# derinworks/penr-oz-neural-network-torch

Hardware: AMD Instinct MI355X
Metric: training samples/sec (whole node), 4x8192 MLP bf16 at 1/2/4/8 MI355X (higher is better)
Workload: dtype bf16; 1 GPU; model=mlp[1024,4096,4096,1024] relu,relu,softmax (25.2M params), global_batch=8192, per_gpu_batch=8192, parallelism=dp1, optimizer=adam, dist_backend=none, dist_world_size=1, launcher=none, config_key=mlp4, engine=fused, grad_dtype=bf16

## Files before the change

penr_oz_neural_network_torch_amd/csrc/bindings.cpp:

```cpp
#include <fcntl.h>
#include <sys/mman.h>
#include <sys/stat.h>
#include <unistd.h>
#include <ATen/ATen.h>
#include <c10/hip/HIPStream.h>
#include <algorithm>
#include <map>
#include <mutex>

#include <torch/library.h>

#include <cstdint>
#include <cstdio>
#include <cstring>
#include <limits>
#include <tuple>
#include <vector>

#include "gemm_dispatch.h"
#include "gemm_sk_plan.h"
#include "json_format.h"
#include "pz_kernels.h"

namespace {
// ... 552 lines not shown
}

void stage_fwd_op(const Tensor& x, const Tensor& y, at::IntArrayRef ei, at::ArrayRef<double> ef) {
  check_dev(x, "x");
  TORCH_CHECK(x.is_contiguous() && y.is_contiguous() && x.numel() == y.numel(), "pz::stage_fwd: contiguous x/y");
  PZ_HIP_CHECK(pz::stage_fwd(x.data_ptr(), dt_of(x), y.data_ptr(), dt_of(y), x.numel(), make_epi(ei, ef), cur_stream(x)));
}

void stage_bwd_op(const Tensor& g, const Tensor& y, const Tensor& dx, at::IntArrayRef ei, at::ArrayRef<double> ef) {
  check_dev(g, "g");
  TORCH_CHECK(g.is_contiguous() && y.is_contiguous() && dx.is_contiguous(), "pz::stage_bwd: contiguous tensors");
  TORCH_CHECK(g.scalar_type() == y.scalar_type() && g.scalar_type() == dx.scalar_type(), "pz::stage_bwd: dtypes");
  TORCH_CHECK(y.is_cuda() && dx.is_cuda() && y.numel() == g.numel() && dx.numel() == g.numel(),
              "pz::stage_bwd: g, y and dx must be GPU tensors of one size");
  PZ_HIP_CHECK(pz::stage_bwd(g.data_ptr(), y.data_ptr(), dx.data_ptr(), dt_of(g), g.numel(), make_epi(ei, ef),
                             cur_stream(g)));
}

void xent_head_op(const Tensor& logits, const Tensor& labels, int64_t rows_valid, const optional<Tensor>& loss,
                  double loss_scale, const optional<Tensor>& dh, double grad_scale, const optional<Tensor>& colsum,
                  const optional<Tensor>& probs, at::IntArrayRef ei, at::ArrayRef<double> ef, int64_t idx_ld,
                  const optional<Tensor>& out8, const optional<Tensor>& out8_qscale, const optional<Tensor>& amax,
                  bool store_dh, const optional<Tensor>& su_amax, const optional<Tensor>& su_qs, double su_headroom,
                  double su_maxval, const optional<Tensor>& su_qs_prev) {
  check_dev(logits, "logits");
  TORCH_CHECK(logits.dim() == 2 && logits.stride(1) == 1, "pz::xent_head: 2-D logits");
  TORCH_CHECK(labels.scalar_type() == at::kLong && labels.is_contiguous(), "pz::xent_head: int64 labels");
  pz::XentArgs a{};
  a.logits = logits.data_ptr();
  a.ld = logits.stride(0);
  a.labels = labels.data_ptr<int64_t>();
  a.rows = static_cast<int>(logits.size(0));
  TORCH_CHECK(rows_valid >= 0 && rows_valid <= logits.size(0), "pz::xent_head: rows_valid ", rows_valid,
              " is outside [0, ", logits.size(0), "]");
  TORCH_CHECK(labels.is_cuda() && labels.numel() >= rows_valid, "pz::xent_head: labels must hold rows_valid entries");
  a.rows_valid = static_cast<int>(rows_valid);
  a.cols = static_cast<int>(logits.size(1));
  a.dtype = dt_of(logits);
  head_accumulators(a, loss, colsum, a.dtype == pz::DT_F64, "pz::xent_head");
  at::Tensor cs_ws;
  if (a.colsum != nullptr && a.dtype == pz::DT_BF16 && pz::deterministic()) {
    const int blocks = (a.rows + 31) / 32, groups = (blocks + 15) / 16;
    cs_ws = at::empty({static_cast<int64_t>(blocks + groups) * a.cols}, logits.options().dtype(at::kFloat));
    a.cs_ws = cs_ws.data_ptr<float>();
    a.cs_tickets = split_counters(groups + 1, logits.device());
  }
  a.loss_scale = loss_scale;
  if (dh.has_value() && dh->defined()) {
    a.dh = opt_mat(dh, logits, a.rows, a.cols, "pz::xent_head", "dh");
// ... 6 lines not shown
  }
  a.epi = make_epi(ei, ef);
  a.idx_ld = idx_ld > 0 ? idx_ld : a.cols;
  if (out8.has_value() && out8->defined()) {
    TORCH_CHECK(out8->scalar_type() == at::kFloat8_e5m2 && out8->dim() == 2 && out8->stride(1) == 1 &&
                    out8->size(0) >= a.rows && out8->size(1) >= a.cols,
                "pz::xent_head: out8 must be float8_e5m2 [rows, cols]");
    a.out8 = static_cast<uint8_t*>(out8->data_ptr());
    a.ld_out8 = out8->stride(0);
    a.out8_qscale = f32_scalar_ptr(out8_qscale, "out8_qscale");
    TORCH_CHECK(a.out8_qscale != nullptr, "pz::xent_head: out8 needs out8_qscale");
    a.amax = opt_vec<float>(amax, at::kFloat, 1, "pz::xent_head", "amax");
  }
  a.skip_dh = store_dh ? 0 : 1;
  a.su = scale_upd(su_amax, su_qs, su_headroom, su_maxval);
  if (su_qs_prev.has_value() && su_qs_prev->defined()) {
    TORCH_CHECK(a.su.n > 0 && su_qs_prev->scalar_type() == at::kFloat && su_qs_prev->is_contiguous() &&
                    su_qs_prev->numel() >= 2 * a.su.n && su_qs_prev->data_ptr<float>() != a.su.qs,
                "pz::xent_head: su_qs_prev: fp32 qs[2n] of the current step, not su_qs itself");
    a.su.qs_prev = su_qs_prev->data_ptr<float>();
  }
  TORCH_CHECK((a.out8 == nullptr && !a.skip_dh) || pz::xent_head_out8_ok(a),
              "pz::xent_head: out8 / store_dh=False need the bf16 fast path (bf16, cols % 8 == 0, <= 2048, aligned)");
  PZ_HIP_CHECK(pz::xent_head(a, cur_stream(logits)));
}

void mse_head_op(const Tensor& y, const Tensor& target, int64_t rows_valid, const optional<Tensor>& loss,
                 double loss_scale, const optional<Tensor>& dh, double grad_scale, const optional<Tensor>& colsum,
                 at::IntArrayRef ei, at::ArrayRef<double> ef, int64_t idx_ld) {
  check_dev(y, "y");
  TORCH_CHECK(y.dim() == 2 && target.dim() == 2 && y.stride(1) == 1 && target.stride(1) == 1, "pz::mse_head: 2-D");
  TORCH_CHECK(y.scalar_type() == target.scalar_type(), "pz::mse_head: dtype mismatch");
  TORCH_CHECK(rows_valid >= 0 && rows_valid <= y.size(0), "pz::mse_head: rows_valid ", rows_valid, " is outside [0, ",
              y.size(0), "]");
  TORCH_CHECK(target.is_cuda() && target.size(0) >= rows_valid && target.size(1) >= y.size(1),
              "pz::mse_head: target must hold [rows_valid, cols]");
  pz::MseArgs a{};
  a.y = y.data_ptr();
  a.ld_y = y.stride(0);
  a.target = target.data_ptr();
  a.ld_t = target.stride(0);
  a.rows = static_cast<int>(y.size(0));
  a.rows_valid = static_cast<int>(rows_valid);
  a.cols = static_cast<int>(y.size(1));
  a.dtype = dt_of(y);
  head_accumulators(a, loss, colsum, a.dtype == pz::DT_F64, "pz::mse_head");
  a.loss_scale = loss_scale;
// ... 762 lines not shown
        "Tensor(a!) params, Tensor(b!)? exp_avg, Tensor(c!)? exp_avg_sq, Tensor(d!)? shadow, Tensor(e!)? stats, "
        "Tensor(f!)? amax, bool adam, float lr, float beta1, float beta2, float eps, float bias_c1, "
        "float bias_c2_sqrt, float grad_scale, float l2, Tensor? hp=None, Tensor? epoch=None, int stats_every=1) -> ()");
  m.def("gemm_path(Tensor A, bool a_kc, Tensor B, bool b_kc, Tensor C, int M, int N, int K, "
        "bool force_generic=False) -> int");
  m.def("gemm_skinny(Tensor x, Tensor w, Tensor(a!) out, Tensor? bias, int act) -> ()");
  m.def("gemm_skinny_eligible(Tensor x, Tensor w, Tensor out) -> bool");
  m.def("gemm_skinny_w8(Tensor x, Tensor w8, Tensor scale, Tensor(a!) out, Tensor? bias, int act) -> ()");
  m.def("gemm_skinny_w8_eligible(Tensor x, Tensor w8, Tensor scale, Tensor out) -> bool");
  m.def("gemm_skinny_plan(int K, int N, int dtype) -> int[]");
  m.def("gemm_skinny_w8_plan(int K, int N) -> int[]");
  m.def("gemm_sk_plan(int M, int N, int K, int cus, int M1=0, int N1=0) -> int[]");
  m.def("gemm_pair_split(Tensor A0, Tensor B0, Tensor C0, Tensor A1, Tensor B1, Tensor C1, int M0, int N0, int M1, "
        "int N1, int K, int engine=0) -> int");
  m.def("gemm_pair(Tensor A0, Tensor B0, Tensor(a!) C0, Tensor A1, Tensor B1, Tensor(b!) C1, int M0, int N0, int M1, "
        "int N1, int K, Tensor? scale_a0=None, Tensor? scale_b0=None, Tensor? scale_a1=None, "
        "Tensor? scale_b1=None, int flags=0) -> ()");
  m.def("stage_fwd(Tensor x, Tensor(a!) y, int[] epi_i, float[] epi_f) -> ()");
  m.def("stage_bwd(Tensor g, Tensor y, Tensor(a!) dx, int[] epi_i, float[] epi_f) -> ()");
  m.def("xent_head(Tensor logits, Tensor labels, int rows_valid, Tensor(a!)? loss, float loss_scale, Tensor(b!)? dh, "
        "float grad_scale, Tensor(c!)? colsum, Tensor(d!)? probs, int[] epi_i, float[] epi_f, int idx_ld, "
        "Tensor(e!)? out8=None, Tensor? out8_qscale=None, Tensor(f!)? amax=None, bool store_dh=True, "
        "Tensor(s!)? su_amax=None, Tensor(t!)? su_qs=None, float su_headroom=1.0, float su_maxval=448.0, "
        "Tensor? su_qs_prev=None) -> ()");
  m.def("mse_head(Tensor y, Tensor target, int rows_valid, Tensor(a!)? loss, float loss_scale, Tensor(b!)? dh, "
        "float grad_scale, Tensor(c!)? colsum, int[] epi_i, float[] epi_f, int idx_ld) -> ()");
  m.def("softmax_rows(Tensor x, Tensor(a!) y) -> ()");
  m.def("sample_rows(Tensor logits, Tensor(a!) seq, Tensor(b!) done, int pos, float temperature, int top_k, int key, "
        "int stop_token=-1, int row0=0, float top_p=1.0, float min_p=0.0) -> ()");
  m.def("generate_resident(Tensor(a!) seq, Tensor(b!) done, Tensor[] params, int[] plan, int steps, float temperature, "
        "int top_k, int seed_lo, int seed_hi, int stop_token=-1, int row0=0, Tensor(c!)? logits_out=None, float top_p=1.0, "
        "float min_p=0.0) -> ()");
  m.def("token_logprob(Tensor logits, Tensor targets, Tensor(a!) logprob, Tensor(b!)? rank) -> ()");
  m.def("topk_rows(Tensor logits, int k, Tensor(a!) idx, Tensor(b!) logprob) -> ()");
  m.def("softmax_bwd(Tensor g, Tensor y, Tensor(a!) dx) -> ()");
  m.def("colsum(Tensor x, Tensor(a!) out) -> ()");
  m.def("gather_rows(Tensor data, Tensor? indices, int seed_lo, int seed_hi, Tensor(a!) out, int rows_valid, "
        "Tensor? labels_in, Tensor(b!)? labels_out, Tensor(c!)? picked, Tensor? epoch=None, Tensor? data8=None, "
        "Tensor(d!)? out8=None, Tensor(s!)? su_amax=None, Tensor(t!)? su_qs=None, float su_headroom=1.0, "
        "float su_maxval=448.0) -> ()");
  m.def("pack_segments(int[] offsets, int[] numels, int[] is_weight, int[] stat_slot, Tensor?[] shadows, "
        "Tensor?[] grads16, int[] zero_grad, Tensor?[] amax, Tensor?[] w8, Tensor?[] w8_amax_prev, "
        "Tensor?[] w8_qs) -> Tensor");
  m.def("optimizer_step(Tensor(a!) params, Tensor(e!) grads, Tensor(b!)? exp_avg, Tensor(c!)? exp_avg_sq, Tensor segments, "
        "Tensor block_seg, int num_segments, int total_blocks, bool adam, float lr, float beta1, float beta2, float eps, "
        "float bias_c1, float bias_c2_sqrt, float grad_scale, float l2, Tensor(d!)? stats, Tensor? hp=None, "
        "Tensor? epoch=None, int stats_every=1, int max_grid=0) -> ()");
// ... 82 lines not shown
```

penr_oz_neural_network_torch_amd/csrc/elementwise.hip:

```cpp
#include "pz_common.h"
#include "pz_launch.h"
#include "pz_kernels.h"

namespace pz {
namespace {

template <typename T> PZ_DEV double ldd(const T* p, int64_t i) { return static_cast<double>(p[i]); }
template <> PZ_DEV double ldd<uint16_t>(const uint16_t* p, int64_t i) { return bf2f(p[i]); }
template <typename T> PZ_DEV void std_(T* p, int64_t i, double v) { p[i] = static_cast<T>(v); }
template <> PZ_DEV void std_<uint16_t>(uint16_t* p, int64_t i, double v) { p[i] = f2bf(static_cast<float>(v)); }

template <typename Tin, typename Tout, typename F>
__global__ void __launch_bounds__(256) stage_fwd_kernel(const Tin* __restrict__ x, Tout* __restrict__ y,
                                                        int64_t n, EpiSpec e) {
  e = epi_resolve(e);
  for (int64_t i = blockIdx.x * int64_t(256) + threadIdx.x; i < n; i += int64_t(gridDim.x) * 256) {
    const F v = static_cast<F>(ldd<Tin>(x, i));
    std_<Tout>(y, i, static_cast<double>(epi_fwd<F>(v, static_cast<uint64_t>(i), e)));
  }
}

template <typename T, typename F>
__global__ void __launch_bounds__(256) stage_bwd_kernel(const T* __restrict__ g, const T* __restrict__ y,
                                                        T* __restrict__ dx, int64_t n, EpiSpec e) {
// ... 26 lines not shown
  if (threadIdx.x == 0) atomicAdd(loss + (slots > 1 ? blockIdx.x % slots : 0), red[0] + red[1] + red[2] + red[3]);
}

template <typename A>
PZ_DEV void block_colsum_flush(A* colsum, const A* cs, int cols) {
  __syncthreads();
  for (int c = threadIdx.x; c < cols; c += 256)
    if (cs[c] != A(0)) atomicAdd(colsum + c, cs[c]);
}

template <int WAVES>
PZ_DEV void head_colsum_flush(const XentArgs& a, const float* cs_lds) {
  __shared__ int det_flag;
  for (int c = threadIdx.x; c < a.cols; c += WAVES * 64) {
    float t = 0.f;
#pragma unroll
    for (int w = 0; w < WAVES; ++w) t += cs_lds[w * a.cols + c];
    if (a.cs_ws != nullptr) st_wt(a.cs_ws + static_cast<int64_t>(blockIdx.x) * a.cols + c, t);
    else if (t != 0.f) atomicAdd(a.colsum + c, t);
  }
  if (a.cs_ws != nullptr)
    det_colsum<WAVES * 64>(a.cs_ws, a.cs_tickets, gridDim.x, 16, blockIdx.x, a.cols, a.cols, a.colsum,
                           (PZ_LDS int*)(&det_flag));
}

template <typename F> PZ_DEV F* head_loss(void* f32, void* f64);
template <> PZ_DEV float* head_loss<float>(void* f32, void*) { return static_cast<float*>(f32); }
template <> PZ_DEV double* head_loss<double>(void*, void* f64) { return static_cast<double*>(f64); }

template <typename T, typename F>
__global__ void __launch_bounds__(256) xent_head_kernel(XentArgs a) {
  apply_scale_update(a.su);
  a.epi = epi_resolve(a.epi);
  extern __shared__ __attribute__((aligned(16))) char cs_raw[];
  F* cs_lds = reinterpret_cast<F*>(cs_raw);
  __shared__ F red[4];
  F* const loss = head_loss<F>(a.loss, a.loss64);
  F* const colsum = head_loss<F>(a.colsum, a.colsum64);
  const T* __restrict__ logits = static_cast<const T*>(a.logits);
  T* __restrict__ dh = static_cast<T*>(a.dh);
  T* __restrict__ probs = static_cast<T*>(a.probs);
  const int lane = threadIdx.x & 63;
  const int wave = threadIdx.x >> 6;
  const bool cs_on = colsum != nullptr && dh != nullptr;
  if (cs_on) {
    for (int c = threadIdx.x; c < a.cols; c += 256) cs_lds[c] = F(0);
// ... 279 lines not shown
  A s = A(0);
  if (c < cols)
    for (int r = r0 + (threadIdx.x >> 6); r < r1; r += 4) s += static_cast<A>(ldd<T>(x, static_cast<int64_t>(r) * ld + c));
  __shared__ A part[4][64];
  part[threadIdx.x >> 6][threadIdx.x & 63] = s;
  __syncthreads();
  if (threadIdx.x < 64 && c < cols) {
    const A v = part[0][threadIdx.x] + part[1][threadIdx.x] + part[2][threadIdx.x] + part[3][threadIdx.x];
    if (ws != nullptr) ws[static_cast<int64_t>(blockIdx.y) * cols + c] = v;
    else atomicAdd(out + c, v);
  }
}

template <typename A>
__global__ void __launch_bounds__(256) colsum_fold_kernel(const A* __restrict__ ws, A* __restrict__ out, int parts,
                                                          int cols) {
  const int c = blockIdx.x * 256 + threadIdx.x;
  if (c >= cols) return;
  A s = A(0);
  for (int y = 0; y < parts; ++y) s += ws[static_cast<int64_t>(y) * cols + c];
  out[c] += s;
}

template <int NCH, int WAVES, bool COLSUM, bool OUT8, bool DROP>
__global__ void __launch_bounds__(WAVES * 64) xent_head_lean_kernel(XentArgs a) {
  apply_scale_update(a.su);
  const EpiSpec e = epi_resolve(a.epi);
  extern __shared__ float cs_lds[];
  __shared__ float red[WAVES];
  constexpr int RPW = kBf16HeadRows / WAVES;
  const uint16_t* __restrict__ logits = static_cast<const uint16_t*>(a.logits);
  uint16_t* __restrict__ dh = static_cast<uint16_t*>(a.dh);
  const int lane = threadIdx.x & 63;
  const int wave = threadIdx.x >> 6;
  float cs[NCH][8];
#pragma unroll
  for (int j = 0; j < NCH; ++j)
#pragma unroll
    for (int q = 0; q < 8; ++q) cs[j][q] = 0.f;
  const int row0 = blockIdx.x * kBf16HeadRows + wave * RPW;
  uint4 raw[RPW][NCH];
  int labels[RPW];
#pragma unroll
  for (int rr = 0; rr < RPW; ++rr) {
    const int row = row0 + rr;
    labels[rr] = row < a.rows_valid ? static_cast<int>(a.labels[row]) : -1;
#pragma unroll
    for (int j = 0; j < NCH; ++j)
      raw[rr][j] = row < a.rows_valid ? *reinterpret_cast<const uint4*>(logits + static_cast<int64_t>(row) * a.ld + (lane + 64 * j) * 8)
                                      : make_uint4(0, 0, 0, 0);
  }
  const float gs = static_cast<float>(a.grad_scale);
  const float qs8 = OUT8 ? *a.out8_qscale : 1.f;
  float loss_acc = 0.f, amax8 = 0.f;
#pragma unroll
  for (int rr = 0; rr < RPW; ++rr) {
    const int row = row0 + rr;
    if (row >= a.rows) break;
    const bool valid = row < a.rows_valid;
    const int label = labels[rr];
    float v[NCH][8];
#pragma unroll
    for (int j = 0; j < NCH; ++j) {
      const uint32_t w[4] = {raw[rr][j].x, raw[rr][j].y, raw[rr][j].z, raw[rr][j].w};
#pragma unroll
      for (int q = 0; q < 4; ++q) { v[j][2 * q] = bf2f(w[q] & 0xFFFF); v[j][2 * q + 1] = bf2f(w[q] >> 16); }
    }
    float mx = -INFINITY, xl = 0.f;
#pragma unroll
    for (int j = 0; j < NCH; ++j)
#pragma unroll
      for (int q = 0; q < 8; ++q) {
        mx = fmaxf(mx, v[j][q]);
        xl += (lane + 64 * j) * 8 + q == label ? v[j][q] : 0.f;
      }
    mx = wave_max(mx);
    float se = 0.f;
#pragma unroll
    for (int j = 0; j < NCH; ++j)
#pragma unroll
      for (int q = 0; q < 8; ++q) {
        v[j][q] = __expf(v[j][q] - mx);
        se += v[j][q];
      }
    se = wave_sum(se);
    xl = wave_sum(xl);
    if (valid && lane == 0) loss_acc += (mx + __logf(se) - xl) * static_cast<float>(a.loss_scale);
    const float inv = valid ? gs / se : 0.f;
    const uint64_t row_idx = static_cast<uint64_t>(row) * static_cast<uint64_t>(a.idx_ld);
#pragma unroll
    for (int j = 0; j < NCH; ++j) {
      const int c0 = (lane + 64 * j) * 8;
      float g[8];
#pragma unroll
      for (int q = 0; q < 8; ++q) g[q] = v[j][q] * inv - (c0 + q == label && valid ? gs : 0.f);
      if constexpr (DROP) {
        const uint32_t p0 = static_cast<uint32_t>((row_idx + c0) >> 1);
#pragma unroll
        for (int h = 0; h < 4; ++h) {
          const uint32_t b = mix32((p0 + h) ^ e.key_pre);
          g[2 * h] = (b & 0xFFFFu) >= e.thresh16 ? g[2 * h] * e.scale : 0.f;
          g[2 * h + 1] = (b >> 16) >= e.thresh16 ? g[2 * h + 1] * e.scale : 0.f;
        }
      }
      const uint4 gb = make_uint4(pack_bf2(g[0], g[1]), pack_bf2(g[2], g[3]), pack_bf2(g[4], g[5]), pack_bf2(g[6], g[7]));
      if (!a.skip_dh) *reinterpret_cast<uint4*>(dh + static_cast<int64_t>(row) * a.ld_dh + c0) = gb;
      if constexpr (OUT8) {
        const uint32_t w[4] = {gb.x, gb.y, gb.z, gb.w};
        float x[8];
#pragma unroll
        for (int q = 0; q < 4; ++q) {
          x[2 * q] = bf2f(w[q] & 0xFFFFu);
          x[2 * q + 1] = bf2f(w[q] >> 16);
          amax8 = fmaxf(amax8, fmaxf(fabsf(x[2 * q]), fabsf(x[2 * q + 1])));
        }
        *reinterpret_cast<u32x2_t*>(a.out8 + static_cast<int64_t>(row) * a.ld_out8 + c0) = to_e5m2x8(x, qs8);
      }
      if constexpr (COLSUM) {
#pragma unroll
        for (int q = 0; q < 8; ++q) cs[j][q] += g[q];
      }
    }
  }
  if constexpr (OUT8) {
    if (a.amax != nullptr) {
      __shared__ float red8[WAVES];
      const float m = wave_max(amax8);
      if (lane == 0) red8[wave] = m;
      __syncthreads();
      if (threadIdx.x == 0) {
        float t = red8[0];
#pragma unroll
        for (int w = 1; w < WAVES; ++w) t = fmaxf(t, red8[w]);
        atomicMax(reinterpret_cast<unsigned int*>(a.amax), __float_as_uint(t));
      }
    }
  }
  if (a.loss != nullptr) {
    const float t = wave_sum(loss_acc);
    if (lane == 0) red[wave] = t;
    __syncthreads();
    if (threadIdx.x == 0) {
      float s = 0.f;
#pragma unroll
      for (int w = 0; w < WAVES; ++w) s += red[w];
      atomicAdd(a.loss + (a.loss_slots > 1 ? blockIdx.x % a.loss_slots : 0), s);
    }
  }
  if constexpr (COLSUM) {
    float* mine = cs_lds + wave * a.cols;
#pragma unroll
    for (int j = 0; j < NCH; ++j)
#pragma unroll
      for (int q = 0; q < 8; ++q) mine[(lane + 64 * j) * 8 + q] = cs[j][q];
    __syncthreads();
    head_colsum_flush<WAVES>(a, cs_lds);
  }
}

template <typename Tin, typename Tout>
__global__ void __launch_bounds__(256) gather_rows_kernel(GatherArgs a) {
  apply_scale_update(a.su);
  if (a.epoch_ptr != nullptr) gather_seed(a.seed_lo, a.seed_hi, static_cast<uint32_t>(*a.epoch_ptr));
  const Tin* __restrict__ src = static_cast<const Tin*>(a.data);
  Tout* __restrict__ dst = static_cast<Tout*>(a.out);
  const int row = blockIdx.x;
  int64_t pick = 0;
  if (row < a.rows_valid) {
    if (a.indices != nullptr) {
      pick = a.indices[row];
    } else {
      const uint32_t h = mix32(mix32(static_cast<uint32_t>(row) ^ a.seed_lo) ^ a.seed_hi);
      pick = static_cast<int64_t>((static_cast<uint64_t>(h) * static_cast<uint64_t>(a.n_data)) >> 32);
    }
    if (threadIdx.x == 0) {
      if (a.picked != nullptr) a.picked[row] = pick;
      if (a.labels_out != nullptr) a.labels_out[row] = a.labels_in[pick];
    }
  } else if (threadIdx.x == 0 && a.labels_out != nullptr) {
// ... 83 lines not shown
  if (n <= 0) return hipSuccess;
  PZ_DISPATCH_FLOAT(dtype, T, {
    using F = typename MathOf<T>::type;
    hipLaunchKernelGGL((stage_bwd_kernel<T, F>), dim3(grid_for(n)), dim3(256), 0, s, static_cast<const T*>(g),
                       static_cast<const T*>(y), static_cast<T*>(dx), n, e);
  });
  return hipGetLastError();
}

template <int NCH, int W, int RPB = kBf16HeadRows>
hipError_t launch_xent_bf16(const XentArgs& a, dim3 grid, size_t lds, hipStream_t s) {
  static bool attr = false;
  if (!attr) {
    hipError_t e = hipFuncSetAttribute(reinterpret_cast<const void*>(xent_head_bf16_kernel<NCH, W, RPB>),
                                       hipFuncAttributeMaxDynamicSharedMemorySize, W * 512 * NCH * 4);
    if (e != hipSuccess) return e;
    attr = true;
  }
  hipLaunchKernelGGL((xent_head_bf16_kernel<NCH, W, RPB>), grid, dim3(W * 64), lds, s, a);
  return hipGetLastError();
}

template <int NCH, bool CS, bool O8, bool DR>
hipError_t launch_xent_lean1(const XentArgs& a, dim3 grid, size_t lds, hipStream_t s) {
  constexpr int W = 16;
  static bool attr = false;
  if (!attr) {
    hipError_t e = hipFuncSetAttribute(reinterpret_cast<const void*>(xent_head_lean_kernel<NCH, W, CS, O8, DR>),
                                       hipFuncAttributeMaxDynamicSharedMemorySize, W * 512 * NCH * 4);
    if (e != hipSuccess) return e;
    attr = true;
  }
  hipLaunchKernelGGL((xent_head_lean_kernel<NCH, W, CS, O8, DR>), grid, dim3(W * 64), lds, s, a);
  return hipGetLastError();
}
template <int NCH>
hipError_t launch_xent_lean_n(const XentArgs& a, bool cs, bool o8, bool dr, dim3 grid, size_t lds, hipStream_t s) {
  if (cs) {
    if (o8) return dr ? launch_xent_lean1<NCH, true, true, true>(a, grid, lds, s) : launch_xent_lean1<NCH, true, true, false>(a, grid, lds, s);
    return dr ? launch_xent_lean1<NCH, true, false, true>(a, grid, lds, s) : launch_xent_lean1<NCH, true, false, false>(a, grid, lds, s);
  }
  if (o8) return dr ? launch_xent_lean1<NCH, false, true, true>(a, grid, lds, s) : launch_xent_lean1<NCH, false, true, false>(a, grid, lds, s);
  return dr ? launch_xent_lean1<NCH, false, false, true>(a, grid, lds, s) : launch_xent_lean1<NCH, false, false, false>(a, grid, lds, s);
}
hipError_t launch_xent_lean(const XentArgs& a, int nch, bool cs, bool o8, bool dr, dim3 grid, size_t lds, hipStream_t s) {
  if (nch == 1) return launch_xent_lean_n<1>(a, cs, o8, dr, grid, lds, s);
  if (nch == 2) return launch_xent_lean_n<2>(a, cs, o8, dr, grid, lds, s);
  return launch_xent_lean_n<4>(a, cs, o8, dr, grid, lds, s);
}

constexpr int kMaxLdsCols = 16384;

bool xent_head_out8_ok(const XentArgs& a) {
  return a.dtype == DT_BF16 && a.cols % 8 == 0 && a.cols <= 2048 && a.ld % 8 == 0 && a.dh != nullptr &&
         a.ld_dh % 8 == 0 && (a.probs == nullptr || a.ld_probs % 8 == 0) && a.idx_ld % 2 == 0 &&
         (reinterpret_cast<uintptr_t>(a.logits) & 15) == 0 && (reinterpret_cast<uintptr_t>(a.dh) & 15) == 0 &&
         (reinterpret_cast<uintptr_t>(a.probs) & 15) == 0 && (a.out8 == nullptr || (a.ld_out8 % 8 == 0 &&
         (reinterpret_cast<uintptr_t>(a.out8) & 7) == 0 && a.out8_qscale != nullptr));
}

hipError_t xent_head(const XentArgs& in, hipStream_t s) {
  if (in.rows <= 0) return hipSuccess;
  XentArgs a = in;
  if ((a.out8 != nullptr || a.skip_dh) && !xent_head_out8_ok(a)) return hipErrorInvalidValue;
  void* colsum_direct = nullptr;
  const bool acc64 = a.dtype == DT_F64;
  if ((a.colsum != nullptr || a.colsum64 != nullptr) && a.cols > kMaxLdsCols / (acc64 ? 2 : 1)) {
    colsum_direct = acc64 ? static_cast<void*>(a.colsum64) : static_cast<void*>(a.colsum);
    a.colsum = nullptr;
    a.colsum64 = nullptr;
  }
  const size_t lds = (acc64 ? a.colsum64 != nullptr : a.colsum != nullptr) ? (acc64 ? 8 : 4) * a.cols : 0;
  const dim3 grid((a.rows + kHeadRows - 1) / kHeadRows);
  const bool vec = a.dtype == DT_BF16 && a.cols % 8 == 0 && a.ld % 8 == 0 && (a.dh == nullptr || a.ld_dh % 8 == 0) &&
                   (a.probs == nullptr || a.ld_probs % 8 == 0) && a.idx_ld % 2 == 0 &&
                   (reinterpret_cast<uintptr_t>(a.logits) & 15) == 0 && (reinterpret_cast<uintptr_t>(a.dh) & 15) == 0 &&
                   (reinterpret_cast<uintptr_t>(a.probs) & 15) == 0;
  const dim3 grid16((a.rows + kBf16HeadRows - 1) / kBf16HeadRows);
  constexpr int kW = 16;
  const size_t ldsw = kW * lds;
  hipError_t le = hipSuccess;
  if (!vec || a.cols > 2048) a.cs_ws = nullptr;
  const EpiSpec& ep = a.epi;
  const int nch = a.cols / 512;
  if (vec && a.probs == nullptr && a.dh != nullptr && a.cols % 512 == 0 && nch >= 1 && nch <= 4 &&
      nch != 3 && ep.act == ACT_NONE && !ep.drop_post && !ep.drop_all && a.labels != nullptr &&
      (a.out8 == nullptr || xent_head_out8_ok(a))) {
    const bool cs = a.colsum != nullptr, o8 = a.out8 != nullptr, dr = ep.drop_pre != 0;
    return launch_xent_lean(a, nch, cs, o8, dr, grid16, cs ? ldsw : 0, s);
  }
  if (vec && a.cols <= 512) le = launch_xent_bf16<1, kW>(a, grid16, ldsw, s);
  else if (vec && a.cols <= 1024) le = launch_xent_bf16<2, kW>(a, grid16, ldsw, s);
  else if (vec && a.cols <= 2048) le = launch_xent_bf16<4, kW>(a, grid16, ldsw, s);
  else {
    PZ_DISPATCH_FLOAT(a.dtype, T, {
      using F = typename MathOf<T>::type;
      hipLaunchKernelGGL((xent_head_kernel<T, F>), grid, dim3(256), lds, s, a);
    });
  }
  if (le != hipSuccess) return le;
  if (colsum_direct != nullptr && a.dh != nullptr) {
    hipError_t e = hipGetLastError();
    if (e != hipSuccess) return e;
    return colsum(a.dh, a.dtype, colsum_direct, acc64 ? DT_F64 : DT_F32, a.rows, a.cols, s, nullptr, a.ld_dh);
  }
  return hipGetLastError();
}

hipError_t mse_head(const MseArgs& in, hipStream_t s) {
  if (in.rows <= 0 || in.cols <= 0) return hipSuccess;
  MseArgs a = in;
  void* colsum_direct = nullptr;
// ... 88 lines not shown
```

penr_oz_neural_network_torch_amd/csrc/optim.hip:

```cpp
#include <cstdlib>

#include "pz_common.h"
#include "pz_kernels.h"

namespace pz {
namespace {

constexpr int kThreads = 256;
constexpr int kPerThread = kOptElemsPerBlock / kThreads;
constexpr float kE4m3Max = 448.f;

PZ_DEV uint32_t e4m3x4(float a, float b, float c, float d) {
  auto sat = [](float x) { return fminf(fmaxf(x, -kE4m3Max), kE4m3Max); };
  uint32_t w = __builtin_amdgcn_cvt_pk_fp8_f32(sat(a), sat(b), 0, false);
  w = __builtin_amdgcn_cvt_pk_fp8_f32(sat(c), sat(d), w, true);
  return w;
}

PZ_DEV int find_segment(const int64_t* block_seg, int nseg, int block) {
  int lo = 0, hi = nseg - 1;
  while (lo < hi) {
    const int mid = (lo + hi + 1) >> 1;
    if (block_seg[mid] <= block) lo = mid; else hi = mid - 1;
  }
// ... 260 lines not shown
__global__ void __launch_bounds__(kThreads) segment_stats_kernel(const R* __restrict__ params,
                                                                 const OptSegment* segments, const int64_t* block_seg,
                                                                 int nseg, double* stats) {
  const int seg_id = find_segment(block_seg, nseg, blockIdx.x);
  const OptSegment seg = segments[seg_id];
  if (seg.stat_slot < 0) return;
  const int64_t local0 = (static_cast<int64_t>(blockIdx.x) - block_seg[seg_id]) * kOptElemsPerBlock;
  double st[4] = {0.0, 0.0, 0.0, 0.0};
  for (int u = 0; u < kPerThread; ++u) {
    const int64_t li = local0 + static_cast<int64_t>(u) * kThreads + threadIdx.x;
    if (li >= seg.numel) break;
    const double w = params[seg.offset + li];
    st[2] += w; st[3] += w * w;
  }
  block_reduce_add(st, stats + 4 * seg.stat_slot);
}

PZ_DEV double std_from_sums(double s, double ss, double n) {
  if (n < 2) return NAN;
  const double var = (ss - s * s / n) / (n - 1.0);
  return sqrt(var > 0.0 ? var : 0.0);
}

__global__ void step_finalize_kernel(FinalizeArgs a) {
  __shared__ double l2sum;
  if (a.epoch < 0) a.epoch = *a.epoch_ptr;
  if (a.ratio_row == -2) a.ratio_row = a.epoch % a.every == 0 ? a.epoch / a.every : -1;
  if (a.ratio_row >= a.n_ratio_rows) a.ratio_row = -1;
  __syncthreads();
  if (threadIdx.x == 0) l2sum = 0.0;
  __syncthreads();
  for (int k = threadIdx.x; k < a.nslots; k += blockDim.x) {
    atomicAdd(&l2sum, a.stats_prev[4 * k + 3]);
    if (a.ratio_row >= 0) {
      const double n = a.slot_numel[k];
      const double* c = a.stats_cur + 4 * k;
      const double sd = std_from_sums(c[0], c[1], n);
      const double sw = std_from_sums(c[2], c[3], n);
      a.ratios[static_cast<int64_t>(a.ratio_row) * a.nslots + k] = static_cast<float>(sd / (sw + 1e-8));
    }
  }
  __syncthreads();
  if (threadIdx.x == 0) {
    double loss = 0.0;
    if (a.loss64 != nullptr) {
      for (int k = 0; k < a.loss_slots; ++k) {
        loss += a.loss64[k];
        a.loss64[k] = 0.0;
      }
      loss /= a.loss_div;
    } else if (a.loss != nullptr) {
      for (int k = 0; k < a.loss_slots; ++k) {
        loss += static_cast<double>(a.loss[k]);
        a.loss[k] = 0.f;
      }
      loss /= a.loss_div;
    }
    if (a.epoch < a.n_costs) a.costs[a.epoch] = loss + static_cast<double>(a.l2) * l2sum;
    if (a.epoch_ptr != nullptr) *a.epoch_ptr = a.epoch + 1;
  }
  __syncthreads();
  for (int k = threadIdx.x; k < 4 * a.nslots; k += blockDim.x) a.stats_prev[k] = 0.0;
  for (int k = threadIdx.x; k < a.nclear; k += blockDim.x) a.clear[k] = 0.f;
}

}

hipError_t step_finalize(const FinalizeArgs& a, hipStream_t s) {
  hipLaunchKernelGGL(step_finalize_kernel, dim3(1), dim3(64), 0, s, a);
  return hipGetLastError();
}

hipError_t optimizer_step(const OptArgs& a, hipStream_t s) {
  if (a.total_blocks <= 0) return hipSuccess;
  const int cap = a.max_grid;
  const int grid = cap > 0 && cap < a.total_blocks ? cap : a.total_blocks;
// ... 24 lines not shown
```

penr_oz_neural_network_torch_amd/csrc/pz_kernels.h:

```cpp
#pragma once

#include "pz_launch.h"

namespace pz {

struct ScaleUpd {
  float* amax;
  float* qs;
  int n;
  float headroom, maxval;
  const float* qs_prev;
};

struct XentArgs {
  const void* logits;
  int64_t ld;
  const int64_t* labels;
  int rows, rows_valid, cols;
  int dtype;
  float* loss;
  double* loss64;
  int loss_slots;
  double loss_scale;
  void* dh;
// ... 41 lines not shown
  int64_t ld_data;
  int data_dtype;
  int64_t n_data;
  const int64_t* indices;
  uint32_t seed_lo, seed_hi;
  void* out;
  int64_t ld_out;
  int out_dtype;
  int rows, rows_valid, cols;
  const int64_t* labels_in;
  int64_t* labels_out;
  int64_t* picked;
  const int* epoch_ptr;
  const uint8_t* data8;
  int64_t ld_data8;
  uint8_t* out8;
  int64_t ld_out8;
  ScaleUpd su;
};


hipError_t stage_fwd(const void* x, int x_dtype, void* y, int y_dtype, int64_t n, const EpiSpec& e, hipStream_t s);
hipError_t stage_bwd(const void* g, const void* y, void* dx, int dtype, int64_t n, const EpiSpec& e, hipStream_t s);
hipError_t xent_head(const XentArgs& a, hipStream_t s);
hipError_t mse_head(const MseArgs& a, hipStream_t s);
hipError_t softmax_rows(const void* x, void* y, int dtype, int rows, int cols, hipStream_t s);
hipError_t softmax_bwd(const void* g, const void* y, void* dx, int dtype, int rows, int cols, hipStream_t s);
constexpr int kSampleMaxCols = 1 << 30;
struct SampleArgs {
  const float* logits;
  int rows, cols;
  int64_t* seq;
  int64_t seq_ld, pos;
  int* done;
  float temperature;
  int top_k;
  float top_p;
  float min_p;
  uint32_t key;
  uint32_t row0;
  int64_t stop_token;
};
hipError_t sample_rows(const SampleArgs& a, hipStream_t s);
constexpr int kSampleNarrowCols = 8192;
constexpr int kSampleScratchBytes = 16912;

constexpr int kTokenLogprobWaveCols = 1024;
// ... 199 lines not shown
```

Before: 7.492 million samples/s.

## Make lean xent head kernel persistent with prefetch and ticketed colsum flush

The lean bf16 cross-entropy head kernel becomes a persistent grid-stride kernel sized to resident occupancy. It prefetches the next row group's logits while computing the current one, and flushes loss and column sums per group through a ticketed deterministic fold that defers one dh store. The step-finalize kernel also replaces a shared-memory double atomic with staged loads and a serial sum on thread 0. This adds per-group synchronisation and register pressure from double buffering, and it touches a head kernel that is a small part of an MLP step dominated by GEMMs.

```diff
diff --git a/penr_oz_neural_network_torch_amd/csrc/bindings.cpp b/penr_oz_neural_network_torch_amd/csrc/bindings.cpp
--- a/penr_oz_neural_network_torch_amd/csrc/bindings.cpp
+++ b/penr_oz_neural_network_torch_amd/csrc/bindings.cpp
@@ -598,9 +598,10 @@
                   const optional<Tensor>& probs, at::IntArrayRef ei, at::ArrayRef<double> ef, int64_t idx_ld,
                   const optional<Tensor>& out8, const optional<Tensor>& out8_qscale, const optional<Tensor>& amax,
                   bool store_dh, const optional<Tensor>& su_amax, const optional<Tensor>& su_qs, double su_headroom,
-                  double su_maxval, const optional<Tensor>& su_qs_prev) {
+                  double su_maxval, const optional<Tensor>& su_qs_prev, int64_t max_grid) {
   check_dev(logits, "logits");
   TORCH_CHECK(logits.dim() == 2 && logits.stride(1) == 1, "pz::xent_head: 2-D logits");
+  TORCH_CHECK(max_grid >= 0, "pz::xent_head: max_grid >= 0 (0: automatic)");
   TORCH_CHECK(labels.scalar_type() == at::kLong && labels.is_contiguous(), "pz::xent_head: int64 labels");
   pz::XentArgs a{};
   a.logits = logits.data_ptr();
@@ -653,7 +654,7 @@
   }
   TORCH_CHECK((a.out8 == nullptr && !a.skip_dh) || pz::xent_head_out8_ok(a),
               "pz::xent_head: out8 / store_dh=False need the bf16 fast path (bf16, cols % 8 == 0, <= 2048, aligned)");
-  PZ_HIP_CHECK(pz::xent_head(a, cur_stream(logits)));
+  PZ_HIP_CHECK(pz::xent_head(a, cur_stream(logits), static_cast<int>(std::min<int64_t>(max_grid, INT32_MAX))));
 }
 
 void mse_head_op(const Tensor& y, const Tensor& target, int64_t rows_valid, const optional<Tensor>& loss,
@@ -1462,7 +1463,7 @@
         "float grad_scale, Tensor(c!)? colsum, Tensor(d!)? probs, int[] epi_i, float[] epi_f, int idx_ld, "
         "Tensor(e!)? out8=None, Tensor? out8_qscale=None, Tensor(f!)? amax=None, bool store_dh=True, "
         "Tensor(s!)? su_amax=None, Tensor(t!)? su_qs=None, float su_headroom=1.0, float su_maxval=448.0, "
-        "Tensor? su_qs_prev=None) -> ()");
+        "Tensor? su_qs_prev=None, int max_grid=0) -> ()");
   m.def("mse_head(Tensor y, Tensor target, int rows_valid, Tensor(a!)? loss, float loss_scale, Tensor(b!)? dh, "
         "float grad_scale, Tensor(c!)? colsum, int[] epi_i, float[] epi_f, int idx_ld) -> ()");
   m.def("softmax_rows(Tensor x, Tensor(a!) y) -> ()");
diff --git a/penr_oz_neural_network_torch_amd/csrc/elementwise.hip b/penr_oz_neural_network_torch_amd/csrc/elementwise.hip
--- a/penr_oz_neural_network_torch_amd/csrc/elementwise.hip
+++ b/penr_oz_neural_network_torch_amd/csrc/elementwise.hip
@@ -72,6 +72,50 @@
   if (a.cs_ws != nullptr)
     det_colsum<WAVES * 64>(a.cs_ws, a.cs_tickets, gridDim.x, 16, blockIdx.x, a.cols, a.cols, a.colsum,
                            (PZ_LDS int*)(&det_flag));
+}
+
+template <typename Late>
+PZ_DEV bool head_ticket(int* ticket, int expect, PZ_LDS int* flag, Late&& late) {
+  asm volatile("s_waitcnt vmcnt(0)" ::: "memory");
+  __syncthreads();
+  int prev = 0;
+  if (threadIdx.x == 0) prev = __hip_atomic_fetch_add(ticket, 1, __ATOMIC_RELAXED, __HIP_MEMORY_SCOPE_AGENT);
+  late();
+  if (threadIdx.x == 0) {
+    const int last = prev == expect - 1;
+    if (last) __hip_atomic_store(ticket, 0, __ATOMIC_RELAXED, __HIP_MEMORY_SCOPE_AGENT);
+    *flag = last;
+  }
+  __syncthreads();
+  return __builtin_amdgcn_readfirstlane(*flag) != 0;
+}
+
+template <int WAVES, typename Late>
+PZ_DEV void head_colsum_flush_at(const XentArgs& a, const float* cs_lds, int idx, int nparts, Late&& late) {
+  constexpr int NT = WAVES * 64, kGroup = 16;
+  __shared__ int det_flag;
+  PZ_LDS int* flag = (PZ_LDS int*)(&det_flag);
+  if (a.cs_ws == nullptr) late();
+  for (int c = threadIdx.x; c < a.cols; c += NT) {
+    float t = 0.f;
+#pragma unroll
+    for (int w = 0; w < WAVES; ++w) t += cs_lds[w * a.cols + c];
+    if (a.cs_ws != nullptr) st_wt(a.cs_ws + static_cast<int64_t>(idx) * a.cols + c, t);
+    else if (t != 0.f) atomicAdd(a.colsum + c, t);
+  }
+  if (a.cs_ws == nullptr) return;
+  const int64_t ld = a.cols;
+  const int ngroups = (nparts + kGroup - 1) / kGroup;
+  const int g = idx / kGroup, gr0 = g * kGroup, gr1 = min(nparts, gr0 + kGroup);
+  if (!head_ticket(a.cs_tickets + g, gr1 - gr0, flag, late)) return;
+  if (ngroups == 1) {
+    for (int c = threadIdx.x; c < a.cols; c += NT) a.colsum[c] += det_fold(a.cs_ws, ld, 0, nparts, c);
+    return;
+  }
+  for (int c = threadIdx.x; c < a.cols; c += NT)
+    st_wt(a.cs_ws + static_cast<int64_t>(nparts + g) * ld + c, det_fold(a.cs_ws, ld, gr0, gr1, c));
+  if (!det_ticket(a.cs_tickets + ngroups, ngroups, flag)) return;
+  for (int c = threadIdx.x; c < a.cols; c += NT) a.colsum[c] += det_fold(a.cs_ws, ld, nparts, nparts + ngroups, c);
 }
 
 template <typename F> PZ_DEV F* head_loss(void* f32, void* f64);
@@ -397,6 +441,20 @@
   out[c] += s;
 }
 
+template <int NCH, int RPW>
+PZ_DEV void lean_head_load(const XentArgs& a, const uint16_t* __restrict__ logits, int64_t row0, int lane,
+                           uint4 (&raw)[RPW][NCH], int (&labels)[RPW]) {
+#pragma unroll
+  for (int rr = 0; rr < RPW; ++rr) {
+    const int64_t row = row0 + rr;
+    labels[rr] = row < a.rows_valid ? static_cast<int>(a.labels[row]) : -1;
+#pragma unroll
+    for (int j = 0; j < NCH; ++j)
+      raw[rr][j] = row < a.rows_valid ? *reinterpret_cast<const uint4*>(logits + row * a.ld + (lane + 64 * j) * 8)
+                                      : make_uint4(0, 0, 0, 0);
+  }
+}
+
 template <int NCH, int WAVES, bool COLSUM, bool OUT8, bool DROP>
 __global__ void __launch_bounds__(WAVES * 64) xent_head_lean_kernel(XentArgs a) {
   apply_scale_update(a.su);
@@ -408,93 +466,127 @@
   uint16_t* __restrict__ dh = static_cast<uint16_t*>(a.dh);
   const int lane = threadIdx.x & 63;
   const int wave = threadIdx.x >> 6;
-  float cs[NCH][8];
-#pragma unroll
-  for (int j = 0; j < NCH; ++j)
-#pragma unroll
-    for (int q = 0; q < 8; ++q) cs[j][q] = 0.f;
-  const int row0 = blockIdx.x * kBf16HeadRows + wave * RPW;
-  uint4 raw[RPW][NCH];
-  int labels[RPW];
-#pragma unroll
-  for (int rr = 0; rr < RPW; ++rr) {
-    const int row = row0 + rr;
-    labels[rr] = row < a.rows_valid ? static_cast<int>(a.labels[row]) : -1;
-#pragma unroll
-    for (int j = 0; j < NCH; ++j)
-      raw[rr][j] = row < a.rows_valid ? *reinterpret_cast<const uint4*>(logits + static_cast<int64_t>(row) * a.ld + (lane + 64 * j) * 8)
-                                      : make_uint4(0, 0, 0, 0);
-  }
+  const int ngroups = (a.rows + kBf16HeadRows - 1) / kBf16HeadRows;
   const float gs = static_cast<float>(a.grad_scale);
   const float qs8 = OUT8 ? *a.out8_qscale : 1.f;
-  float loss_acc = 0.f, amax8 = 0.f;
-#pragma unroll
-  for (int rr = 0; rr < RPW; ++rr) {
-    const int row = row0 + rr;
-    if (row >= a.rows) break;
-    const bool valid = row < a.rows_valid;
-    const int label = labels[rr];
-    float v[NCH][8];
-#pragma unroll
-    for (int j = 0; j < NCH; ++j) {
-      const uint32_t w[4] = {raw[rr][j].x, raw[rr][j].y, raw[rr][j].z, raw[rr][j].w};
-#pragma unroll
-      for (int q = 0; q < 4; ++q) { v[j][2 * q] = bf2f(w[q] & 0xFFFF); v[j][2 * q + 1] = bf2f(w[q] >> 16); }
-    }
-    float mx = -INFINITY, xl = 0.f;
+  float amax8 = 0.f;
+  uint4 raw[RPW][NCH], nxt[RPW][NCH];
+  int labels[RPW], nlabels[RPW];
+  lean_head_load<NCH, RPW>(a, logits, static_cast<int64_t>(blockIdx.x) * kBf16HeadRows + wave * RPW, lane, raw, labels);
+  for (int rg = blockIdx.x; rg < ngroups; rg += gridDim.x) {
+    const int row0 = rg * kBf16HeadRows + wave * RPW;
+    lean_head_load<NCH, RPW>(a, logits, row0 + static_cast<int64_t>(gridDim.x) * kBf16HeadRows, lane, nxt, nlabels);
+    float cs[NCH][8];
 #pragma unroll
     for (int j = 0; j < NCH; ++j)
 #pragma unroll
-      for (int q = 0; q < 8; ++q) {
-        mx = fmaxf(mx, v[j][q]);
-        xl += (lane + 64 * j) * 8 + q == label ? v[j][q] : 0.f;
+      for (int q = 0; q < 8; ++q) cs[j][q] = 0.f;
+    float loss_acc = 0.f;
+#pragma unroll
+    for (int rr = 0; rr < RPW; ++rr) {
+      const int row = row0 + rr;
+      if (row >= a.rows) break;
+      const bool valid = row < a.rows_valid;
+      const int label = labels[rr];
+      float v[NCH][8];
+#pragma unroll
+      for (int j = 0; j < NCH; ++j) {
+        const uint32_t w[4] = {raw[rr][j].x, raw[rr][j].y, raw[rr][j].z, raw[rr][j].w};
+#pragma unroll
+        for (int q = 0; q < 4; ++q) { v[j][2 * q] = bf2f(w[q] & 0xFFFF); v[j][2 * q + 1] = bf2f(w[q] >> 16); }
       }
-    mx = wave_max(mx);
-    float se = 0.f;
-#pragma unroll
-    for (int j = 0; j < NCH; ++j)
-#pragma unroll
-      for (int q = 0; q < 8; ++q) {
-        v[j][q] = __expf(v[j][q] - mx);
-        se += v[j][q];
-      }
-    se = wave_sum(se);
-    xl = wave_sum(xl);
-    if (valid && lane == 0) loss_acc += (mx + __logf(se) - xl) * static_cast<float>(a.loss_scale);
-    const float inv = valid ? gs / se : 0.f;
-    const uint64_t row_idx = static_cast<uint64_t>(row) * static_cast<uint64_t>(a.idx_ld);
-#pragma unroll
-    for (int j = 0; j < NCH; ++j) {
-      const int c0 = (lane + 64 * j) * 8;
-      float g[8];
-#pragma unroll
-      for (int q = 0; q < 8; ++q) g[q] = v[j][q] * inv - (c0 + q == label && valid ? gs : 0.f);
-      if constexpr (DROP) {
-        const uint32_t p0 = static_cast<uint32_t>((row_idx + c0) >> 1);
-#pragma unroll
-        for (int h = 0; h < 4; ++h) {
-          const uint32_t b = mix32((p0 + h) ^ e.key_pre);
-          g[2 * h] = (b & 0xFFFFu) >= e.thresh16 ? g[2 * h] * e.scale : 0.f;
-          g[2 * h + 1] = (b >> 16) >= e.thresh16 ? g[2 * h + 1] * e.scale : 0.f;
+      float mx = -INFINITY, xl = 0.f;
+#pragma unroll
+      for (int j = 0; j < NCH; ++j)
+#pragma unroll
+        for (int q = 0; q < 8; ++q) {
+          mx = fmaxf(mx, v[j][q]);
+          xl += (lane + 64 * j) * 8 + q == label ? v[j][q] : 0.f;
+        }
+      mx = wave_max(mx);
+      float se = 0.f;
+#pragma unroll
+      for (int j = 0; j < NCH; ++j)
+#pragma unroll
+        for (int q = 0; q < 8; ++q) {
+          v[j][q] = __expf(v[j][q] - mx);
+          se += v[j][q];
+        }
+      se = wave_sum(se);
+      xl = wave_sum(xl);
+      if (valid && lane == 0) loss_acc += (mx + __logf(se) - xl) * static_cast<float>(a.loss_scale);
+      const float inv = valid ? gs / se : 0.f;
+      const uint64_t row_idx = static_cast<uint64_t>(row) * static_cast<uint64_t>(a.idx_ld);
+#pragma unroll
+      for (int j = 0; j < NCH; ++j) {
+        const int c0 = (lane + 64 * j) * 8;
+        float g[8];
+#pragma unroll
+        for (int q = 0; q < 8; ++q) g[q] = v[j][q] * inv - (c0 + q == label && valid ? gs : 0.f);
+        if constexpr (DROP) {
+          const uint32_t p0 = static_cast<uint32_t>((row_idx + c0) >> 1);
+#pragma unroll
+          for (int h = 0; h < 4; ++h) {
+            const uint32_t b = mix32((p0 + h) ^ e.key_pre);
+            g[2 * h] = (b & 0xFFFFu) >= e.thresh16 ? g[2 * h] * e.scale : 0.f;
+            g[2 * h + 1] = (b >> 16) >= e.thresh16 ? g[2 * h + 1] * e.scale : 0.f;
+          }
+        }
+        const uint4 gb = make_uint4(pack_bf2(g[0], g[1]), pack_bf2(g[2], g[3]), pack_bf2(g[4], g[5]), pack_bf2(g[6], g[7]));
+        if (COLSUM && rr == RPW - 1) raw[rr][j] = gb;
+        else if (!a.skip_dh) *reinterpret_cast<uint4*>(dh + static_cast<int64_t>(row) * a.ld_dh + c0) = gb;
+        if constexpr (OUT8) {
+          const uint32_t w[4] = {gb.x, gb.y, gb.z, gb.w};
+          float x[8];
+#pragma unroll
+          for (int q = 0; q < 4; ++q) {
+            x[2 * q] = bf2f(w[q] & 0xFFFFu);
+            x[2 * q + 1] = bf2f(w[q] >> 16);
+            amax8 = fmaxf(amax8, fmaxf(fabsf(x[2 * q]), fabsf(x[2 * q + 1])));
+          }
+          *reinterpret_cast<u32x2_t*>(a.out8 + static_cast<int64_t>(row) * a.ld_out8 + c0) = to_e5m2x8(x, qs8);
+        }
+        if constexpr (COLSUM) {
+#pragma unroll
+          for (int q = 0; q < 8; ++q) cs[j][q] += g[q];
         }
       }
-      const uint4 gb = make_uint4(pack_bf2(g[0], g[1]), pack_bf2(g[2], g[3]), pack_bf2(g[4], g[5]), pack_bf2(g[6], g[7]));
-      if (!a.skip_dh) *reinterpret_cast<uint4*>(dh + static_cast<int64_t>(row) * a.ld_dh + c0) = gb;
-      if constexpr (OUT8) {
-        const uint32_t w[4] = {gb.x, gb.y, gb.z, gb.w};
-        float x[8];
-#pragma unroll
-        for (int q = 0; q < 4; ++q) {
-          x[2 * q] = bf2f(w[q] & 0xFFFFu);
-          x[2 * q + 1] = bf2f(w[q] >> 16);
-          amax8 = fmaxf(amax8, fmaxf(fabsf(x[2 * q]), fabsf(x[2 * q + 1])));
-        }
-        *reinterpret_cast<u32x2_t*>(a.out8 + static_cast<int64_t>(row) * a.ld_out8 + c0) = to_e5m2x8(x, qs8);
-      }
-      if constexpr (COLSUM) {
-#pragma unroll
-        for (int q = 0; q < 8; ++q) cs[j][q] += g[q];
-      }
+    }
+    if (a.loss != nullptr) {
+      const float t = wave_sum(loss_acc);
+      if (lane == 0) red[wave] = t;
+    }
+    if constexpr (COLSUM) {
+      float* mine = cs_lds + wave * a.cols;
+#pragma unroll
+      for (int j = 0; j < NCH; ++j)
+#pragma unroll
+        for (int q = 0; q < 8; ++q) mine[(lane + 64 * j) * 8 + q] = cs[j][q];
+    }
+    if (COLSUM || a.loss != nullptr) __syncthreads();
+    if (a.loss != nullptr && threadIdx.x == 0) {
+      float s = 0.f;
+#pragma unroll
+      for (int w = 0; w < WAVES; ++w) s += red[w];
+      atomicAdd(a.loss + (a.loss_slots > 1 ? rg % a.loss_slots : 0), s);
+    }
+    if constexpr (COLSUM) {
+      const auto store_held = [&] {
+        const int row = row0 + RPW - 1;
+        if (row >= a.rows || a.skip_dh) return;
+#pragma unroll
+        for (int j = 0; j < NCH; ++j)
+          *reinterpret_cast<uint4*>(dh + static_cast<int64_t>(row) * a.ld_dh + (lane + 64 * j) * 8) = raw[RPW - 1][j];
+      };
+      head_colsum_flush_at<WAVES>(a, cs_lds, rg, ngroups, store_held);
+    }
+    if (rg + static_cast<int>(gridDim.x) >= ngroups) break;
+    if (COLSUM || a.loss != nullptr) __syncthreads();
+#pragma unroll
+    for (int rr = 0; rr < RPW; ++rr) {
+      labels[rr] = nlabels[rr];
+#pragma unroll
+      for (int j = 0; j < NCH; ++j) raw[rr][j] = nxt[rr][j];
     }
   }
   if constexpr (OUT8) {
@@ -510,26 +602,6 @@
         atomicMax(reinterpret_cast<unsigned int*>(a.amax), __float_as_uint(t));
       }
     }
-  }
-  if (a.loss != nullptr) {
-    const float t = wave_sum(loss_acc);
-    if (lane == 0) red[wave] = t;
-    __syncthreads();
-    if (threadIdx.x == 0) {
-      float s = 0.f;
-#pragma unroll
-      for (int w = 0; w < WAVES; ++w) s += red[w];
-      atomicAdd(a.loss + (a.loss_slots > 1 ? blockIdx.x % a.loss_slots : 0), s);
-    }
-  }
-  if constexpr (COLSUM) {
-    float* mine = cs_lds + wave * a.cols;
-#pragma unroll
-    for (int j = 0; j < NCH; ++j)
-#pragma unroll
-      for (int q = 0; q < 8; ++q) mine[(lane + 64 * j) * 8 + q] = cs[j][q];
-    __syncthreads();
-    head_colsum_flush<WAVES>(a, cs_lds);
   }
 }
 
@@ -659,31 +731,39 @@
 }
 
 template <int NCH, bool CS, bool O8, bool DR>
-hipError_t launch_xent_lean1(const XentArgs& a, dim3 grid, size_t lds, hipStream_t s) {
+hipError_t launch_xent_lean1(const XentArgs& a, int max_grid, size_t lds, hipStream_t s) {
   constexpr int W = 16;
-  static bool attr = false;
-  if (!attr) {
-    hipError_t e = hipFuncSetAttribute(reinterpret_cast<const void*>(xent_head_lean_kernel<NCH, W, CS, O8, DR>),
-                                       hipFuncAttributeMaxDynamicSharedMemorySize, W * 512 * NCH * 4);
+  static int resident = 0;
+  if (resident == 0) {
+    const void* fn = reinterpret_cast<const void*>(xent_head_lean_kernel<NCH, W, CS, O8, DR>);
+    hipError_t e = hipFuncSetAttribute(fn, hipFuncAttributeMaxDynamicSharedMemorySize, W * 512 * NCH * 4);
     if (e != hipSuccess) return e;
-    attr = true;
-  }
-  hipLaunchKernelGGL((xent_head_lean_kernel<NCH, W, CS, O8, DR>), grid, dim3(W * 64), lds, s, a);
+    int dev = 0, cus = 0, per_cu = 0;
+    if ((e = hipGetDevice(&dev)) != hipSuccess) return e;
+    if ((e = hipDeviceGetAttribute(&cus, hipDeviceAttributeMultiprocessorCount, dev)) != hipSuccess) return e;
+    e = hipOccupancyMaxActiveBlocksPerMultiprocessor(&per_cu, xent_head_lean_kernel<NCH, W, CS, O8, DR>, W * 64, lds);
+    if (e != hipSuccess) return e;
+    if (cus < 1 || per_cu < 1) return hipErrorLaunchOutOfResources;
+    resident = cus * per_cu;
+  }
+  const int groups = (a.rows + kBf16HeadRows - 1) / kBf16HeadRows;
+  const int grid = max_grid > 0 ? (max_grid < groups ? max_grid : groups) : (groups < resident ? groups : resident);
+  hipLaunchKernelGGL((xent_head_lean_kernel<NCH, W, CS, O8, DR>), dim3(grid), dim3(W * 64), lds, s, a);
   return hipGetLastError();
 }
 template <int NCH>
-hipError_t launch_xent_lean_n(const XentArgs& a, bool cs, bool o8, bool dr, dim3 grid, size_t lds, hipStream_t s) {
+hipError_t launch_xent_lean_n(const XentArgs& a, bool cs, bool o8, bool dr, int max_grid, size_t lds, hipStream_t s) {
   if (cs) {
-    if (o8) return dr ? launch_xent_lean1<NCH, true, true, true>(a, grid, lds, s) : launch_xent_lean1<NCH, true, true, false>(a, grid, lds, s);
-    return dr ? launch_xent_lean1<NCH, true, false, true>(a, grid, lds, s) : launch_xent_lean1<NCH, true, false, false>(a, grid, lds, s);
-  }
-  if (o8) return dr ? launch_xent_lean1<NCH, false, true, true>(a, grid, lds, s) : launch_xent_lean1<NCH, false, true, false>(a, grid, lds, s);
-  return dr ? launch_xent_lean1<NCH, false, false, true>(a, grid, lds, s) : launch_xent_lean1<NCH, false, false, false>(a, grid, lds, s);
-}
-hipError_t launch_xent_lean(const XentArgs& a, int nch, bool cs, bool o8, bool dr, dim3 grid, size_t lds, hipStream_t s) {
-  if (nch == 1) return launch_xent_lean_n<1>(a, cs, o8, dr, grid, lds, s);
-  if (nch == 2) return launch_xent_lean_n<2>(a, cs, o8, dr, grid, lds, s);
-  return launch_xent_lean_n<4>(a, cs, o8, dr, grid, lds, s);
+    if (o8) return dr ? launch_xent_lean1<NCH, true, true, true>(a, max_grid, lds, s) : launch_xent_lean1<NCH, true, true, false>(a, max_grid, lds, s);
+    return dr ? launch_xent_lean1<NCH, true, false, true>(a, max_grid, lds, s) : launch_xent_lean1<NCH, true, false, false>(a, max_grid, lds, s);
+  }
+  if (o8) return dr ? launch_xent_lean1<NCH, false, true, true>(a, max_grid, lds, s) : launch_xent_lean1<NCH, false, true, false>(a, max_grid, lds, s);
+  return dr ? launch_xent_lean1<NCH, false, false, true>(a, max_grid, lds, s) : launch_xent_lean1<NCH, false, false, false>(a, max_grid, lds, s);
+}
+hipError_t launch_xent_lean(const XentArgs& a, int nch, bool cs, bool o8, bool dr, int max_grid, size_t lds, hipStream_t s) {
+  if (nch == 1) return launch_xent_lean_n<1>(a, cs, o8, dr, max_grid, lds, s);
+  if (nch == 2) return launch_xent_lean_n<2>(a, cs, o8, dr, max_grid, lds, s);
+  return launch_xent_lean_n<4>(a, cs, o8, dr, max_grid, lds, s);
 }
 
 constexpr int kMaxLdsCols = 16384;
@@ -696,7 +776,7 @@
          (reinterpret_cast<uintptr_t>(a.out8) & 7) == 0 && a.out8_qscale != nullptr));
 }
 
-hipError_t xent_head(const XentArgs& in, hipStream_t s) {
+hipError_t xent_head(const XentArgs& in, hipStream_t s, int max_grid) {
   if (in.rows <= 0) return hipSuccess;
   XentArgs a = in;
   if ((a.out8 != nullptr || a.skip_dh) && !xent_head_out8_ok(a)) return hipErrorInvalidValue;
@@ -724,7 +804,7 @@
       nch != 3 && ep.act == ACT_NONE && !ep.drop_post && !ep.drop_all && a.labels != nullptr &&
       (a.out8 == nullptr || xent_head_out8_ok(a))) {
     const bool cs = a.colsum != nullptr, o8 = a.out8 != nullptr, dr = ep.drop_pre != 0;
-    return launch_xent_lean(a, nch, cs, o8, dr, grid16, cs ? ldsw : 0, s);
+    return launch_xent_lean(a, nch, cs, o8, dr, max_grid, cs ? ldsw : 0, s);
   }
   if (vec && a.cols <= 512) le = launch_xent_bf16<1, kW>(a, grid16, ldsw, s);
   else if (vec && a.cols <= 1024) le = launch_xent_bf16<2, kW>(a, grid16, ldsw, s);
diff --git a/penr_oz_neural_network_torch_amd/csrc/optim.hip b/penr_oz_neural_network_torch_amd/csrc/optim.hip
--- a/penr_oz_neural_network_torch_amd/csrc/optim.hip
+++ b/penr_oz_neural_network_torch_amd/csrc/optim.hip
@@ -306,16 +306,19 @@
   return sqrt(var > 0.0 ? var : 0.0);
 }
 
+constexpr int kFinalizeStage = 64;
 __global__ void step_finalize_kernel(FinalizeArgs a) {
-  __shared__ double l2sum;
+  __shared__ double sq_stage[kFinalizeStage], loss_stage[kFinalizeStage];
   if (a.epoch < 0) a.epoch = *a.epoch_ptr;
   if (a.ratio_row == -2) a.ratio_row = a.epoch % a.every == 0 ? a.epoch / a.every : -1;
   if (a.ratio_row >= a.n_ratio_rows) a.ratio_row = -1;
-  __syncthreads();
-  if (threadIdx.x == 0) l2sum = 0.0;
+  for (int k = threadIdx.x; k < a.nslots && k < kFinalizeStage; k += blockDim.x) sq_stage[k] = a.stats_prev[4 * k + 3];
+  for (int k = threadIdx.x; k < a.loss_slots && k < kFinalizeStage; k += blockDim.x) {
+    if (a.loss64 != nullptr) loss_stage[k] = a.loss64[k];
+    else if (a.loss != nullptr) loss_stage[k] = static_cast<double>(a.loss[k]);
+  }
   __syncthreads();
   for (int k = threadIdx.x; k < a.nslots; k += blockDim.x) {
-    atomicAdd(&l2sum, a.stats_prev[4 * k + 3]);
     if (a.ratio_row >= 0) {
       const double n = a.slot_numel[k];
       const double* c = a.stats_cur + 4 * k;
@@ -324,18 +327,19 @@
       a.ratios[static_cast<int64_t>(a.ratio_row) * a.nslots + k] = static_cast<float>(sd / (sw + 1e-8));
     }
   }
-  __syncthreads();
   if (threadIdx.x == 0) {
+    double l2sum = 0.0;
+    for (int k = 0; k < a.nslots; ++k) l2sum += k < kFinalizeStage ? sq_stage[k] : a.stats_prev[4 * k + 3];
     double loss = 0.0;
     if (a.loss64 != nullptr) {
       for (int k = 0; k < a.loss_slots; ++k) {
-        loss += a.loss64[k];
+        loss += k < kFinalizeStage ? loss_stage[k] : a.loss64[k];
         a.loss64[k] = 0.0;
       }
       loss /= a.loss_div;
     } else if (a.loss != nullptr) {
       for (int k = 0; k < a.loss_slots; ++k) {
-        loss += static_cast<double>(a.loss[k]);
+        loss += k < kFinalizeStage ? loss_stage[k] : static_cast<double>(a.loss[k]);
         a.loss[k] = 0.f;
       }
       loss /= a.loss_div;
diff --git a/penr_oz_neural_network_torch_amd/csrc/pz_kernels.h b/penr_oz_neural_network_torch_amd/csrc/pz_kernels.h
--- a/penr_oz_neural_network_torch_amd/csrc/pz_kernels.h
+++ b/penr_oz_neural_network_torch_amd/csrc/pz_kernels.h
@@ -87,7 +87,7 @@
 
 hipError_t stage_fwd(const void* x, int x_dtype, void* y, int y_dtype, int64_t n, const EpiSpec& e, hipStream_t s);
 hipError_t stage_bwd(const void* g, const void* y, void* dx, int dtype, int64_t n, const EpiSpec& e, hipStream_t s);
-hipError_t xent_head(const XentArgs& a, hipStream_t s);
+hipError_t xent_head(const XentArgs& a, hipStream_t s, int max_grid = 0);
 hipError_t mse_head(const MseArgs& a, hipStream_t s);
 hipError_t softmax_rows(const void* x, void* y, int dtype, int rows, int cols, hipStream_t s);
 hipError_t softmax_bwd(const void* g, const void* y, void* dx, int dtype, int rows, int cols, hipStream_t s);
```

Measured after the change: 7.486 million samples/s. Within noise of the previous version (-0.1%).
